# nh2/lz4-frame-conduit

Measured on AMD Instinct MI355X. Metric: GiB/s end-to-end (compress+decompress), 4 MiB blocks, 1/2/4/8 GPUs vs liblz4, higher is better.
Workload: dtype u8

## Files before the change

lz4_frame_conduit_amd/csrc/encode.cuh:

```cuda
#pragma once
#include <type_traits>
#include "common.cuh"

namespace lz4f {

constexpr uint32_t MFLIMIT = 12, LASTLIT = 5, MINMATCH = 4;
constexpr uint32_t ENC_POOL_SHORT = 0x200u;

struct ChunkInfo {
    uint32_t nrec;
    uint32_t first_lit;
    uint32_t tail_lit;
    uint32_t body_size;
    uint32_t carry_in;
    uint32_t flags;
    uint64_t out_off;
};

struct EncGeom {
    uint64_t src_size;
    uint64_t first_off;
    uint32_t write_endmark;
    uint32_t block_size;
    uint32_t chunk_size;
    uint32_t chunks_per_block;
    uint32_t n_blocks;
    uint32_t n_chunks;
    uint32_t linked;
    uint32_t block_checksum;
    uint32_t header_size;
    uint8_t  header[20];
    uint32_t max_rec_per_chunk;
    uint64_t rec_pool;
    uint32_t seed_stride;
    uint32_t tiles_per_wg;
    uint32_t e1_solo;
    uint32_t hc_attempts;
    uint32_t hc_lazy;
};

struct EncPlace {
    uint64_t bstart, bend_abs;
    uint64_t cs_abs, ce_abs;
    uint64_t low_abs;
    uint64_t rd_end;
};
__device__ __forceinline__ bool enc_place(const EncGeom& g, uint32_t chunk, EncPlace& pl)
{
    const uint32_t blk = chunk / g.chunks_per_block, cib = chunk % g.chunks_per_block;
    pl.bstart = g.first_off + (uint64_t)blk * g.block_size;
    pl.bend_abs = (pl.bstart + g.block_size < g.src_size) ? pl.bstart + g.block_size : g.src_size;
    pl.cs_abs = pl.bstart + (uint64_t)cib * g.chunk_size;
    if (pl.cs_abs >= pl.bend_abs) return false;
    pl.ce_abs = (pl.cs_abs + g.chunk_size < pl.bend_abs) ? pl.cs_abs + g.chunk_size : pl.bend_abs;
    pl.low_abs = g.linked ? 0 : pl.bstart;
    pl.rd_end = g.src_size;
    return true;
}

__device__ __forceinline__ unsigned long long* rec_ctl(const uint64_t* recs) { return (unsigned long long*)recs; }
__device__ __forceinline__ uint32_t* rec_offs(const uint64_t* recs) { return (uint32_t*)(recs + 8); }
__host__ __device__ __forceinline__ uint64_t rec_pool_at(uint32_t n_chunks) { return 8 + (((uint64_t)n_chunks + 1 + 15) / 16) * 8; }
__device__ __forceinline__ uint64_t* rec_pool_of(const uint64_t* recs, const EncGeom& g) { return (uint64_t*)recs + rec_pool_at(g.n_chunks); }

__device__ __forceinline__ uint32_t len_ext_bytes(uint32_t v) { return v >= 15 ? (v - 15) / 255 + 1 : 0; }
__device__ __forceinline__ uint32_t seq_size(uint32_t lit, uint32_t mlen)
{
    return 1 + len_ext_bytes(lit) + lit + 2 + len_ext_bytes(mlen - MINMATCH);
}
__device__ __forceinline__ uint64_t pack_rec(uint32_t lit, uint32_t mlen, uint32_t off)
{
    return (uint64_t)lit | ((uint64_t)mlen << 24) | ((uint64_t)off << 48);
}

struct uint4_ua { uint32_t x, y, z, w; } __attribute__((packed, aligned(1)));
__device__ __forceinline__ uint32_t ld32(const uint8_t* p) { return *(const u32_ua*)p; }
typedef uint64_t u64_ua __attribute__((aligned(1)));
__device__ __forceinline__ uint64_t ld64_guard(const uint8_t* p, const uint8_t* end)
{
    if (p + 8 <= end) return *(const u64_ua*)p;
    uint64_t v = 0;
    for (int i = 0; i < 8; i++) if (p + i < end) v |= (uint64_t)p[i] << (8 * i);
    return v;
}

constexpr uint32_t E1_TILE = 65536, E1_RING = 2 * E1_TILE, E1_RMASK = E1_RING - 1;
#ifndef E1_SLICE_BYTES
#define E1_SLICE_BYTES 128
#endif
constexpr uint32_t E1_SLICE = E1_SLICE_BYTES, E1_NSLICE = E1_TILE / E1_SLICE, E1_REC_PER_SLICE = E1_SLICE / MINMATCH;
constexpr uint32_t E1_HASH_LOG = 13;
#ifndef E1_WAVES
#define E1_WAVES 16
#endif
#ifdef E1_DEBUG
#define E1DBG(...) __VA_ARGS__
#else
#define E1DBG(...)
#endif
#define E1_DBG_AT (((uint64_t)gridDim.x) * (2 * E1_NSLICE * E1_REC_PER_SLICE))
struct alignas(16) E1Shared {
    uint16_t table[1u << E1_HASH_LOG];
    uint8_t  tags[1u << E1_HASH_LOG];
    uint32_t s_end[2][E1_NSLICE];
    uint8_t  s_n[2][E1_NSLICE];
    uint32_t next, cov;
    uint32_t first;
    uint32_t cur[16];
    uint32_t pieces[2];
    uint32_t mode, hits;
    uint32_t tail_d[2];
    uint32_t idle[64];
    alignas(16) uint8_t ring[E1_RING + 16];
};
static_assert(sizeof(E1Shared) <= 163840, "one workgroup per CU");
static_assert(64 * E1_WAVES >= E1_NSLICE, "a thread per slice when the lists are merged");
#ifndef E1_GRAB
#define E1_GRAB 8
#endif
#ifndef E1_GRAB_D
#define E1_GRAB_D 1
#endif
#ifndef E1_DENSE_PASS
#define E1_DENSE_PASS 1
#endif
#ifndef E1_V2
#define E1_V2 1
#endif
#ifndef E1_V3
#define E1_V3 1
#endif
#ifndef E1_V4
#define E1_V4 1
#endif
#ifndef E1_STEP0
#define E1_STEP0 4
#endif
#ifndef E1_IP2
#define E1_IP2 0
#endif
#ifndef E1_OPENER
#define E1_OPENER 2
#endif
#ifndef E1_ALIGN
#define E1_ALIGN 1
#endif
#ifndef E1_STEP_HIT
#define E1_STEP_HIT 1
#endif
constexpr uint32_t E1_GRAB_SPARSE = E1_GRAB, E1_GRAB_DENSE = E1_GRAB_D, E1_PROBE_SLICES = 16, E1_DENSE_HITS = 24;

struct __attribute__((aligned(4))) e1_w2 { uint32_t a, b; };
struct __attribute__((aligned(4))) e1_w3 { uint32_t a, b, c; };
__device__ __forceinline__ uint32_t e1_ld32(const uint8_t* ring, uint32_t pos)
{
    const uint32_t i = pos & E1_RMASK;
    const e1_w2 w = *(const e1_w2*)(ring + (i & ~3u));
    return __builtin_amdgcn_alignbyte(w.b, w.a, i & 3u);
}
__device__ __forceinline__ uint64_t e1_ld64(const uint8_t* ring, uint32_t pos)
{
    const uint32_t i = pos & E1_RMASK;
    const e1_w3 w = *(const e1_w3*)(ring + (i & ~3u));
    return (uint64_t)__builtin_amdgcn_alignbyte(w.b, w.a, i & 3u) | ((uint64_t)__builtin_amdgcn_alignbyte(w.c, w.b, i & 3u) << 32);
}
struct __attribute__((aligned(4))) e1_w5 { uint32_t a, b, c, d, e; };
__device__ __forceinline__ e1_w5 e1_ld5(const uint8_t* ring, uint32_t pos)
{
    return *(const e1_w5*)(ring + ((pos & E1_RMASK) & ~3u));
}
__device__ __forceinline__ uint32_t e1_same16(const e1_w5& s1, const e1_w5& s2, uint32_t k1, uint32_t k2)
{
    const uint32_t x0 = __builtin_amdgcn_alignbyte(s1.b, s1.a, k1) ^ __builtin_amdgcn_alignbyte(s2.b, s2.a, k2);
    const uint32_t x1 = __builtin_amdgcn_alignbyte(s1.c, s1.b, k1) ^ __builtin_amdgcn_alignbyte(s2.c, s2.b, k2);
    const uint32_t x2 = __builtin_amdgcn_alignbyte(s1.d, s1.c, k1) ^ __builtin_amdgcn_alignbyte(s2.d, s2.c, k2);
    const uint32_t x3 = __builtin_amdgcn_alignbyte(s1.e, s1.d, k1) ^ __builtin_amdgcn_alignbyte(s2.e, s2.d, k2);
    const uint64_t lo = (uint64_t)x0 | ((uint64_t)x1 << 32), hi = (uint64_t)x2 | ((uint64_t)x3 << 32);
    return lo ? (uint32_t)(__builtin_ctzll(lo) >> 3) : hi ? 8u + (uint32_t)(__builtin_ctzll(hi) >> 3) : 16u;
}
__device__ __forceinline__ uint32_t e1_mix(uint32_t v) { return v * 2654435761u; }
__device__ __forceinline__ uint32_t e1_slot(uint32_t hv) { return hv >> (32 - E1_HASH_LOG); }
__device__ __forceinline__ uint32_t e1_tag(uint32_t hv) { return (hv >> (24 - E1_HASH_LOG)) & 0xFFu; }
__device__ __forceinline__ uint32_t wave_excl_scan(uint32_t v, uint32_t& total)
{
    const uint32_t lane = lane_id();
    uint32_t incl = v;
#pragma unroll
    for (int sft = 1; sft < 64; sft <<= 1) { const uint32_t t = __shfl_up(incl, sft); if ((int)lane >= sft) incl += t; }
    total = __builtin_amdgcn_readlane(incl, 63);
    return incl - v;
}
__device__ __forceinline__ uint32_t wave_max(uint32_t v)
{
#pragma unroll
    for (int s = 1; s < 64; s <<= 1) { const uint32_t t = __shfl_xor(v, s); v = t > v ? t : v; }
    return v;
}
__device__ __forceinline__ uint32_t wave_sum(uint32_t v)
{
#pragma unroll
    for (int s = 1; s < 64; s <<= 1) v += __shfl_xor(v, s);
    return v;
}
__device__ __forceinline__ uint32_t wave_min16(uint32_t v)
{
    uint32_t t;
    t = (uint32_t)__builtin_amdgcn_update_dpp((int)v, (int)v, 0x111 , 0xf, 0xf, false); v = t < v ? t : v;
    t = (uint32_t)__builtin_amdgcn_update_dpp((int)v, (int)v, 0x112 , 0xf, 0xf, false); v = t < v ? t : v;
    t = (uint32_t)__builtin_amdgcn_update_dpp((int)v, (int)v, 0x114 , 0xf, 0xf, false); v = t < v ? t : v;
    t = (uint32_t)__builtin_amdgcn_update_dpp((int)v, (int)v, 0x118 , 0xf, 0xf, false); v = t < v ? t : v;
    return (uint32_t)__builtin_amdgcn_readlane((int)v, 15);
}
__device__ __forceinline__ uint32_t wave_excl_scan_max(uint32_t v)
{
    const uint32_t lane = lane_id();
    uint32_t incl = v;
#pragma unroll
    for (int sft = 1; sft < 64; sft <<= 1) { const uint32_t t = __shfl_up(incl, sft); if ((int)lane >= sft) incl = t > incl ? t : incl; }
    const uint32_t ex = __shfl_up(incl, 1);
    return lane == 0 ? 0u : ex;
}
constexpr uint32_t E1_PIECE_LOG = 12, E1_NPIECE = E1_TILE >> E1_PIECE_LOG;
__device__ __forceinline__ void e1_dma_piece(E1Shared& sh, const uint8_t* __restrict__ src, uint64_t org, uint32_t nts, uint32_t pc)
{
    const uint32_t lane = lane_id();
    const uint32_t ring0 = (uint32_t)(uintptr_t)(lptr_t)sh.ring;
#pragma unroll
    for (uint32_t q = 0; q < 4; q++) {
        const uint32_t at = nts + (pc << E1_PIECE_LOG) + q * 1024u;
        const uint8_t* gsrc = src + (org + at + lane * 16u);
        const uint32_t ldst = uni(ring0 + (at & E1_RMASK));
        uint32_t keep;
        asm volatile("s_mov_b32 %0, m0\n\ts_mov_b32 m0, %2\n\ts_nop 0\n\tglobal_load_lds_dwordx4 %1, off\n\ts_mov_b32 m0, %0" : "=&s"(keep) : "v"(gsrc), "s"(ldst) : "memory");
    }
}

__device__ __forceinline__ void e1_fill(E1Shared& sh, const uint8_t* __restrict__ src, uint64_t org, uint32_t a, uint32_t b, uint32_t tid)
{
    constexpr uint32_t NT = 64 * E1_WAVES;
    auto put = [&](uint32_t p) { const uint8_t v = src[org + p]; sh.ring[p & E1_RMASK] = v; if ((p & E1_RMASK) < 16) sh.ring[E1_RING + (p & E1_RMASK)] = v; };
    const uint32_t a16 = (a + 15u) & ~15u, b16 = b & ~15u;
    if (a16 < b16) {
        for (uint32_t u = a16 + tid * 16; u < b16; u += NT * 16) {
            const b16_ua t = *(const b16_ua*)(src + (org + u));
            const uint32_t i = u & E1_RMASK;
            *(uint4*)(sh.ring + i) = uint4{t.a, t.b, t.c, t.d};
            if (i == 0) *(uint4*)(sh.ring + E1_RING) = uint4{t.a, t.b, t.c, t.d};
        }
        if (tid < a16 - a) put(a + tid);
        if (tid < b - b16) put(b16 + tid);
    } else {
        for (uint32_t p = a + tid; p < b; p += NT) put(p);
    }
}

struct E1Walk {
    uint32_t pos, cov, bend;
    __device__ __forceinline__ bool step(uint64_t x, uint32_t& start, uint32_t& mlen)
    {
        const uint32_t lit = (uint32_t)(x & 0xFFFFFFu); mlen = (uint32_t)((x >> 24) & 0xFFFFFFu);
        start = pos + lit;
        const uint32_t end = start + mlen;
        pos = end;
        if (end <= cov) return false;
        if (start < cov) {
            const uint32_t ml2 = end - cov;
            if (ml2 < MINMATCH || cov + MFLIMIT > bend) return false;
            start = cov; mlen = ml2;
        }
        return true;
    }
};

__global__ __launch_bounds__(64 * E1_WAVES) void k_find_matches(const uint8_t* __restrict__ src, EncGeom g, ChunkInfo* __restrict__ info,
                                                                uint64_t* __restrict__ recs, uint64_t* __restrict__ scratch)
{
    __shared__ E1Shared sh;
    constexpr uint32_t NT = 64 * E1_WAVES;
    const uint32_t tid = threadIdx.x, lane = lane_id(), wave = uni(tid >> 6);
    uint64_t* spec = scratch + (uint64_t)blockIdx.x * (2 * E1_NSLICE * E1_REC_PER_SLICE);
    const uint32_t c0 = blockIdx.x * g.tiles_per_wg;
    const uint32_t c1 = (c0 + g.tiles_per_wg < g.n_chunks) ? c0 + g.tiles_per_wg : g.n_chunks;
    const uint64_t s0 = g.first_off + (uint64_t)c0 * E1_TILE;
    const uint64_t org = s0 - E1_TILE;
    uint32_t hist = 0, len0 = 0;
    if (s0 < g.src_size) {
        const uint64_t bstart0 = g.first_off + (uint64_t)(c0 / g.chunks_per_block) * g.block_size;
        const uint64_t bend0 = (bstart0 + g.block_size < g.src_size) ? bstart0 + g.block_size : g.src_size;
        const uint64_t low_abs = g.linked ? 0 : bstart0;
        hist = (uint32_t)((s0 - low_abs < E1_TILE) ? s0 - low_abs : E1_TILE);
        len0 = (uint32_t)((bend0 - s0 < E1_TILE) ? bend0 - s0 : E1_TILE);
    }
    const uint32_t hist0 = E1_TILE - hist;
    for (uint32_t i = tid; i < (1u << E1_HASH_LOG) / 2; i += NT) ((uint32_t*)sh.table)[i] = 0;
    for (uint32_t i = tid; i < (1u << E1_HASH_LOG) / 4; i += NT) ((uint32_t*)sh.tags)[i] = 0;
    e1_fill(sh, src, org, hist0, E1_TILE + len0, tid);
    __syncthreads();
    const uint32_t nt_seed = (g.e1_solo & 1u) ? WAVE : NT;
    if (tid < nt_seed) for (uint32_t p = hist0 + tid * g.seed_stride; p < E1_TILE; p += nt_seed * g.seed_stride)
        if (p + 4 <= E1_TILE + len0) { const uint32_t hv = e1_mix(e1_ld32(sh.ring, p)); sh.table[e1_slot(hv)] = (uint16_t)p; sh.tags[e1_slot(hv)] = (uint8_t)e1_tag(hv); }

    auto merge = [&](uint32_t c, uint32_t par, uint32_t ts, uint32_t te, uint32_t bend, uint32_t nslice) {
        constexpr uint32_t SP = E1_NSLICE / WAVE;
        const uint32_t* s_end = sh.s_end[par];
        const uint8_t* s_n = sh.s_n[par];
        const uint64_t* spc = spec + (size_t)par * (E1_NSLICE * E1_REC_PER_SLICE);
        const uint32_t s_lo = lane * SP;
        uint32_t lmax = 0;
#pragma unroll
        for (uint32_t j = 0; j < SP; j++) { const uint32_t e = (s_lo + j < nslice) ? s_end[s_lo + j] : 0u; lmax = e > lmax ? e : lmax; }
        uint32_t cov0 = wave_excl_scan_max(lmax);
        if (cov0 < ts) cov0 = ts;
        uint32_t nn[SP]; ulonglong2 x01[SP];
#pragma unroll
        for (uint32_t j = 0; j < SP; j++) nn[j] = (s_lo + j < nslice) ? s_n[s_lo + j] : 0u;
#pragma unroll
        for (uint32_t j = 0; j < SP; j++) x01[j] = *(const ulonglong2*)(spc + (nn[j] ? s_lo + j : 0u) * E1_REC_PER_SLICE);
        uint32_t kept = 0, f_start = 0, f_mlen = 0, last_end = 0, body = 0;
        {
            uint32_t cov = cov0;
#pragma unroll
            for (uint32_t j = 0; j < SP; j++) {
                const uint32_t sj = s_lo + j, n = nn[j];
                const uint64_t* lst = spc + sj * E1_REC_PER_SLICE;
                E1Walk w{ts + sj * E1_SLICE, cov, bend};
                ulonglong2 cur = x01[j];
                for (uint32_t r = 0; r < n; r += 2) {
                    ulonglong2 nx2 = cur;
                    if (r + 2 < n) nx2 = *(const ulonglong2*)(lst + r + 2);
#pragma unroll
                    for (uint32_t h = 0; h < 2; h++) {
                        if (r + h >= n) break;
                        uint32_t st, ml;
                        if (!w.step(h ? cur.y : cur.x, st, ml)) continue;
                        if (kept == 0) { f_start = st; f_mlen = ml; }
                        else body += seq_size(st - last_end, ml);
                        last_end = st + ml; kept++;
                    }
                    cur = nx2;
                }
                const uint32_t e = (sj < nslice) ? s_end[sj] : 0u; cov = e > cov ? e : cov;
            }
        }
        uint32_t ktot;
        uint32_t prev_end = wave_excl_scan_max(last_end);
        const uint32_t off = wave_excl_scan(kept, ktot);
        uint32_t kmax = wave_max(last_end);
        if (prev_end < ts) prev_end = ts;
        if (kmax < ts) kmax = ts;
        const uint32_t f_lit = kept ? f_start - prev_end : 0u;
        if (kept) body += seq_size(f_lit, f_mlen);
        const uint32_t btot = wave_sum(body);
        const uint64_t has = __ballot(kept != 0);
        const uint32_t tile_first = has ? (uint32_t)__builtin_amdgcn_readlane(f_lit, (int)__builtin_ctzll(has)) : 0u;
        unsigned long long base = 0;
        if (lane == 0 && ktot) base = atomicAdd(rec_ctl(recs), (unsigned long long)ktot);
        base = ((unsigned long long)__builtin_amdgcn_readfirstlane((uint32_t)(base >> 32)) << 32) | __builtin_amdgcn_readfirstlane((uint32_t)base);
        const bool room = base + ktot <= g.rec_pool;
        if (!room && lane == 0) atomicAdd(rec_ctl(recs) + 1, 1ull);
        if (room) {
            if (lane == 0) rec_offs(recs)[c] = (uint32_t)base;
            uint64_t* out = rec_pool_of(recs, g) + base + off;
            uint32_t cov = cov0, jn = 0, le = prev_end;
#pragma unroll
            for (uint32_t j = 0; j < SP; j++) {
                const uint32_t sj = s_lo + j, n = nn[j];
                const uint64_t* lst = spc + sj * E1_REC_PER_SLICE;
                E1Walk w{ts + sj * E1_SLICE, cov, bend};
                ulonglong2 cur = x01[j];
                for (uint32_t r = 0; r < n; r += 2) {
                    ulonglong2 nx2 = cur;
                    if (r + 2 < n) nx2 = *(const ulonglong2*)(lst + r + 2);
#pragma unroll
                    for (uint32_t h = 0; h < 2; h++) {
                        if (r + h >= n) break;
                        const uint64_t x = h ? cur.y : cur.x;
                        uint32_t st, ml;
                        if (!w.step(x, st, ml)) continue;
                        out[jn++] = pack_rec(st - le, ml, (uint32_t)(x >> 48));
                        le = st + ml;
                    }
                    cur = nx2;
                }
                const uint32_t e = (sj < nslice) ? s_end[sj] : 0u; cov = e > cov ? e : cov;
            }
        }
        ChunkInfo* ci = info + c;
        if (lane == 0) {
            if (room) { ci->nrec = ktot; ci->first_lit = tile_first; ci->tail_lit = te - kmax; ci->body_size = btot; }
            else      { ci->nrec = 0; ci->first_lit = 0; ci->tail_lit = te - ts; ci->body_size = 0; }
            sh.mode = (uint64_t)ktot * 64 > (uint64_t)(te - ts) ? 2u : 1u;
        }
    };

    if (tid == 0) { sh.mode = 0; sh.cov = E1_TILE; sh.hits = 0; sh.first = 0; sh.next = E1_ALIGN ? 0 : 1; sh.pieces[0] = 0; sh.pieces[1] = 0; sh.tail_d[0] = 0; sh.tail_d[1] = 0; }
    if (tid < 16) sh.cur[tid] = 0;
    uint32_t mode_tile = 0;
    uint32_t hold = 1;
    bool pend = false;
    uint32_t p_c = 0, p_par = 0, p_ts = 0, p_te = 0, p_bend = 0, p_ns = 0;
    __syncthreads();
    for (uint32_t c = c0; c < c1; c++) {
        const uint32_t k = c - c0;
        const uint32_t ts = E1_TILE * (k + 1), par = k & 1u;
        const uint32_t blk = c / g.chunks_per_block;
        const uint64_t bstart = g.first_off + (uint64_t)blk * g.block_size;
        const uint64_t bend_abs = (bstart + g.block_size < g.src_size) ? bstart + g.block_size : g.src_size;
        const uint64_t cs_abs = s0 + (uint64_t)k * E1_TILE;
        if (cs_abs >= bend_abs) {
            ChunkInfo* ci = info + c;
            if (tid == 0) { ci->nrec = 0; ci->first_lit = 0; ci->tail_lit = 0; ci->body_size = 0; }
            continue;
        }
        const uint32_t tlen = (uint32_t)((bend_abs - cs_abs < E1_TILE) ? bend_abs - cs_abs : E1_TILE);
        const uint32_t te = ts + tlen;
        const uint32_t bend = ts + (uint32_t)(bend_abs - cs_abs);
        const uint32_t blen = (uint32_t)(bend_abs - bstart);
        const uint32_t nslice = (tlen + E1_SLICE - 1) / E1_SLICE;
        uint32_t low = hist0;
        if (!g.linked) { const uint64_t back = cs_abs - bstart; if (back < (uint64_t)(ts - hist0)) low = ts - (uint32_t)back; }
        uint64_t* spec_t = spec + (size_t)par * (E1_NSLICE * E1_REC_PER_SLICE);

        uint32_t nlen = 0;
        const uint32_t nts = ts + E1_TILE;
        if (c + 1 < c1) {
            const uint32_t nblk = (c + 1) / g.chunks_per_block;
            const uint64_t nbstart = g.first_off + (uint64_t)nblk * g.block_size;
            const uint64_t nbend = (nbstart + g.block_size < g.src_size) ? nbstart + g.block_size : g.src_size;
            const uint64_t ncs = cs_abs + E1_TILE;
            if (ncs < nbend) nlen = (uint32_t)((nbend - ncs < E1_TILE) ? nbend - ncs : E1_TILE);
        }
        const bool nlen_full = nlen == E1_TILE;

        E1DBG(const unsigned long long q0 = clock64();)
        if (pend && wave == E1_WAVES - 1) {
            *(lane == 0 ? &sh.cur[wave] : &sh.idle[lane]) = 0xFFFFFFFFu;
            merge(p_c, p_par, p_ts, p_te, p_bend, p_ns);
        }

        E1DBG(const unsigned long long q1 = clock64();)
        const uint32_t end_lim = (te < bend - LASTLIT) ? te : bend - LASTLIT;
        E1DBG(uint32_t dq = 0; unsigned long long a_deq = 0, a_probe = 0, a_hit = 0, n_step = 0, n_hit = 0, n_deq = 0;)
        bool fresh = true;
        for (;;) {
            if ((g.e1_solo & 1u) && tid >= WAVE) break;
            E1DBG(const unsigned long long z0 = clock64(); n_deq++;)
            E1DBG(if (++dq > 100000) { if (lane == 0) atomicAdd((unsigned long long*)&scratch[E1_DBG_AT + 0], 1ull); break; })
            uint32_t mode = (g.e1_solo & 1u) ? mode_tile : uni(__hip_atomic_load(&sh.mode, __ATOMIC_RELAXED, __HIP_MEMORY_SCOPE_WORKGROUP));
            const bool opener = fresh && wave == 0 && (!E1_ALIGN || hold);
            const uint32_t grab = opener ? 1u : mode == 1 ? E1_GRAB_SPARSE : mode == 2 ? E1_GRAB_DENSE : 1u;
            uint32_t si = 0;
            if (E1_ALIGN && opener) si = uni(atomicAdd(lane == 0 ? &sh.next : &sh.idle[lane], grab));
            if (!opener) {
                if (fresh && E1_OPENER && ((E1_OPENER == 1 && !E1_ALIGN) || hold)) for (uint32_t spin = 0; spin < 4096 && uni(__hip_atomic_load(&sh.first, __ATOMIC_RELAXED, __HIP_MEMORY_SCOPE_WORKGROUP)) == 0; spin++) __builtin_amdgcn_s_sleep(2);
                si = uni(atomicAdd(lane == 0 ? &sh.next : &sh.idle[lane], grab));
            }
            fresh = false;
            if (si >= nslice) { *(lane == 0 ? &sh.cur[wave] : &sh.idle[lane]) = 0xFFFFFFFFu; break; }
            *(lane == 0 ? &sh.cur[wave] : &sh.idle[lane]) = si;
            if (nlen_full && (si & 31u) < grab) {
                uint32_t mn = lane < E1_WAVES ? __hip_atomic_load(&sh.cur[lane], __ATOMIC_RELAXED, __HIP_MEMORY_SCOPE_WORKGROUP) : 0xFFFFFFFFu;
                mn = wave_min16(mn);
                uint32_t ok_p = mn == 0xFFFFFFFFu ? 0u : (mn * E1_SLICE) >> E1_PIECE_LOG;
                if (ok_p > E1_NPIECE) ok_p = E1_NPIECE;
                const uint32_t had = uni(atomicMax(lane == 0 ? &sh.pieces[par] : &sh.idle[lane], ok_p));
                for (uint32_t pc = had; pc < ok_p; pc++) e1_dma_piece(sh, src, org, ts + E1_TILE, pc);
            }
            if (mode == 0 && si >= 2 * E1_PROBE_SLICES) {
                mode = uni(__hip_atomic_load(&sh.hits, __ATOMIC_RELAXED, __HIP_MEMORY_SCOPE_WORKGROUP)) > E1_DENSE_HITS ? 2u : 1u;
                *(lane == 0 ? &sh.mode : &sh.idle[lane]) = mode;
                mode_tile = mode;
            }
            const uint32_t cs = ts + si * E1_SLICE;
            const uint32_t ce = (cs + grab * E1_SLICE < te) ? cs + grab * E1_SLICE : te;
            uint64_t* myrec = spec_t + si * E1_REC_PER_SLICE;
            E1DBG(a_deq += clock64() - z0;)
            uint32_t nrec = 0, anchor = cs;
            uint32_t ip = uni(__hip_atomic_load(&sh.cov, __ATOMIC_RELAXED, __HIP_MEMORY_SCOPE_WORKGROUP));
            if (ip < cs) ip = cs;
            if (!(g.e1_solo & 2u) && blen >= MFLIMIT + 1 && ip + MINMATCH <= te && ip + MFLIMIT <= bend && ip < ce) {
                uint32_t last_start = ce - 1;
                if (te - MINMATCH < last_start) last_start = te - MINMATCH;
                if (bend - MFLIMIT < last_start) last_start = bend - MFLIMIT;
                const uint32_t floor_b = ip;
                uint32_t step = (E1_STEP0 > 1 && mode == 1 && !opener) ? (uint32_t)E1_STEP0 : 1u, two = opener ? 0u : 1u;
                E1DBG(uint32_t it = 0;)
                while (ip <= last_start) {
                    E1DBG(if (++it > 100000) { if (lane == 0) { atomicAdd((unsigned long long*)&scratch[E1_DBG_AT + 1], 1ull); scratch[E1_DBG_AT + 8] = ((uint64_t)ip << 32) | last_start; scratch[E1_DBG_AT + 9] = ((uint64_t)step << 32) | si; } break; })
                    E1DBG(const unsigned long long z1 = clock64(); n_step++;)
                    const uint32_t ipB = ip + WAVE * step, stepB = step + 1;
                    const uint32_t pA = ip + lane * step, pB = ipB + lane * stepB;
                    const bool actA = pA <= last_start, actB = two && pB <= last_start;
#if E1_V3
                    const uint32_t iA = pA & E1_RMASK, iB = pB & E1_RMASK;
                    const e1_w2 wA = *(const e1_w2*)(sh.ring + (iA & ~3u)), wB = *(const e1_w2*)(sh.ring + (iB & ~3u));
                    __builtin_amdgcn_sched_barrier(0);
                    const uint32_t vA = __builtin_amdgcn_alignbyte(wA.b, wA.a, iA & 3u), vB = __builtin_amdgcn_alignbyte(wB.b, wB.a, iB & 3u);
                    const uint32_t hvA = e1_mix(vA), hA = e1_slot(hvA), tgA = e1_tag(hvA);
                    const uint32_t hvB = e1_mix(vB), hB = e1_slot(hvB), tgB = e1_tag(hvB);
                    const uint32_t eA = sh.table[hA], etA = sh.tags[hA], eB = sh.table[hB], etB = sh.tags[hB];
                    __builtin_amdgcn_sched_barrier(0);
#else
                    const uint32_t vA = e1_ld32(sh.ring, pA), vB = e1_ld32(sh.ring, pB);
                    const uint32_t hvA = e1_mix(vA), hA = e1_slot(hvA), tgA = e1_tag(hvA);
                    const uint32_t hvB = e1_mix(vB), hB = e1_slot(hvB), tgB = e1_tag(hvB);
                    const uint32_t eA = sh.table[hA], etA = sh.tags[hA], eB = sh.table[hB], etB = sh.tags[hB];
#endif
                    const uint32_t distA = (pA - eA) & 0xFFFFu, distB = (pB - eB) & 0xFFFFu;
                    const uint32_t roomA = pA - low, roomB = pB - low;
#if E1_V3
                    const uint32_t xA = (uint32_t)(uint16_t)((uint16_t)distA - (uint16_t)1u) | ((etA ^ tgA) << 20);
                    const uint32_t xB = (uint32_t)(uint16_t)((uint16_t)distB - (uint16_t)1u) | ((etB ^ tgB) << 20);
#else
                    const uint32_t xA = ((distA - 1u) & 0xFFFFu) | ((etA ^ tgA) << 20) | (distA == 0u ? 1u << 19 : 0u);
                    const uint32_t xB = ((distB - 1u) & 0xFFFFu) | ((etB ^ tgB) << 20) | (distB == 0u ? 1u << 19 : 0u);
#endif
                    const uint32_t nbA = (uint32_t)__builtin_amdgcn_update_dpp(0, (int)vA, 0x111 , 0xf, 0xf, E1_V3 ? true : false);
                    const uint32_t nbB = (uint32_t)__builtin_amdgcn_update_dpp(0, (int)vB, 0x111 , 0xf, 0xf, E1_V3 ? true : false);
#if E1_V2
                    const uint64_t actmA = __ballot(pA <= last_start), actmB = __ballot(pB <= last_start) & (two ? ~0ull : 0ull);
                    constexpr uint32_t LIMCAP = E1_V3 ? 65535u : 65536u;
                    const uint32_t limA = roomA < LIMCAP ? roomA : LIMCAP, limB = roomB < LIMCAP ? roomB : LIMCAP;
                    const bool rleA = nbA == vA, rleB = nbB == vB;
                    const uint32_t dA = rleA ? step : distA, dB = rleB ? stepB : distB;
                    const uint32_t yA = rleA ? step - 1u : xA, yB = rleB ? stepB - 1u : xB;
                    uint64_t m = __ballot(yA < limA) & actmA;
                    if (m) m &= __ballot(e1_ld32(sh.ring, pA - dA) == vA);
                    bool inB = false;
                    if (!m) {
                        *(actA ? &sh.table[hA] : (uint16_t*)&sh.idle[lane]) = (uint16_t)pA; *(actA ? &sh.tags[hA] : (uint8_t*)&sh.idle[lane]) = (uint8_t)tgA;
                        m = __ballot(yB < limB) & actmB;
                        if (m) m &= __ballot(e1_ld32(sh.ring, pB - dB) == vB);
                        inB = true;
                    }
#else
                    const uint32_t limA = actA ? (roomA < 65536u ? roomA : 65536u) : 0u, limB = actB ? (roomB < 65536u ? roomB : 65536u) : 0u;
                    const uint32_t row0 = (lane & 15u) == 0u ? 1u : 0u;
                    uint64_t m = __ballot(xA < limA);
                    if (m) m &= __ballot(e1_ld32(sh.ring, pA - distA) == vA);
                    uint64_t mr = __ballot(((nbA ^ vA) | row0 | (actA ? 0u : 1u)) == 0u) & ~m;
                    m |= mr;
                    bool inB = false;
                    if (!m) {
                        *(actA ? &sh.table[hA] : (uint16_t*)&sh.idle[lane]) = (uint16_t)pA; *(actA ? &sh.tags[hA] : (uint8_t*)&sh.idle[lane]) = (uint8_t)tgA;
                        m = __ballot(xB < limB);
                        if (m) m &= __ballot(e1_ld32(sh.ring, pB - distB) == vB);
                        mr = __ballot(((nbB ^ vB) | row0 | (actB ? 0u : 1u)) == 0u) & ~m;
                        m |= mr;
                        inB = true;
                    }
                    const uint32_t dA = ((mr >> lane) & 1ull) ? step : distA, dB = ((mr >> lane) & 1ull) ? stepB : distB;
#endif
                    const uint32_t L = m ? (uint32_t)__builtin_ctzll(m) : WAVE;
                    {
                        const bool ins = (inB ? actB : actA) && lane <= L;
                        const uint32_t hI = inB ? hB : hA, pI = inB ? pB : pA, tI = inB ? tgB : tgA;
                        *(ins ? &sh.table[hI] : (uint16_t*)&sh.idle[lane]) = (uint16_t)pI; *(ins ? &sh.tags[hI] : (uint8_t*)&sh.idle[lane]) = (uint8_t)tI;
                    }
                    E1DBG(const unsigned long long z2 = clock64(); a_probe += z2 - z1;)
                    if (!m) { ip = two ? ipB + WAVE * stepB : ipB; step += 1 + two; two = 1; continue; }
                    E1DBG(n_hit++;)
                    if (E1_DENSE_PASS && !inB && mode == 2 && step == 1) {
                        const uint32_t di = dA;
                        const uint64_t x0 = e1_ld64(sh.ring, pA + 4) ^ e1_ld64(sh.ring, pA + 4 - di);
                        const uint64_t x1 = e1_ld64(sh.ring, pA + 12) ^ e1_ld64(sh.ring, pA + 12 - di);
                        const uint32_t xb = e1_ld32(sh.ring, pA - 4) ^ e1_ld32(sh.ring, pA - 4 - di);
                        const uint32_t g0 = x0 ? (uint32_t)(__builtin_ctzll(x0) >> 3) : 8u, g1 = x1 ? (uint32_t)(__builtin_ctzll(x1) >> 3) : 8u;
                        const uint32_t fraw = 4u + g0 + (g0 == 8u ? g1 : 0u), flim = end_lim - pA;
                        const uint32_t fl = fraw < flim ? fraw : flim;
                        const uint32_t lng = (fraw >= 20u && flim > 20u) ? 1u : 0u;
                        const uint32_t nbk = xb ? (uint32_t)(__builtin_clz(xb) >> 3) : 4u;
                        const uint32_t flx = fl | (lng << 31);
                        if (!((uint32_t)__builtin_amdgcn_readlane((int)flx, (int)L) >> 31)) {
                            uint64_t taken = 0, rem = m;
                            uint32_t endrel = 0, stop_at = WAVE;
                            for (;;) {
                                const uint32_t sx = (uint32_t)__builtin_ctzll(rem);
                                const uint32_t fx = (uint32_t)__builtin_amdgcn_readlane((int)flx, (int)sx);
                                if (fx >> 31) { stop_at = sx; break; }
                                taken |= 1ull << sx;
                                endrel = sx + fx;
                                if (endrel >= WAVE) break;
                                rem &= ~((1ull << endrel) - 1ull);
                                if (!rem) break;
                            }
                            const bool is_t = (taken >> lane) & 1ull;
                            const uint32_t pe = dpp_excl_scan_max(is_t ? lane + fl : 0u);
                            const uint32_t before = pe ? ip + pe : anchor;
                            const uint32_t bfloor = pe ? ip + pe : (anchor > floor_b ? anchor : floor_b);
                            uint32_t nb = nbk;
                            if (pA - bfloor < nb) nb = pA - bfloor;
                            if (pA - di - low < nb) nb = pA - di - low;
                            const uint32_t rank = (uint32_t)__builtin_popcountll(taken & ((1ull << lane) - 1ull));
                            if (is_t) myrec[nrec + rank] = pack_rec(pA - nb - before, fl + nb, di);
                            nrec += (uint32_t)__builtin_popcountll(taken);
                            E1DBG(if (blockIdx.x == 0 && lane == 0) { atomicAdd((unsigned long long*)&scratch[E1_DBG_AT + 13], 1ull); atomicAdd((unsigned long long*)&scratch[E1_DBG_AT + 14], (unsigned long long)__builtin_popcountll(taken)); atomicAdd((unsigned long long*)&scratch[E1_DBG_AT + 15], (unsigned long long)(stop_at < WAVE ? stop_at : (endrel > WAVE ? endrel : WAVE))); })
                            anchor = ip + endrel;
                            const uint32_t nrel = stop_at < WAVE ? stop_at : (endrel > WAVE ? endrel : WAVE);
                            const bool ins2 = actA && lane > L && lane < nrel && lane >= pe;
                            *(ins2 ? &sh.table[hA] : (uint16_t*)&sh.idle[lane]) = (uint16_t)pA; *(ins2 ? &sh.tags[hA] : (uint8_t*)&sh.idle[lane]) = (uint8_t)tgA;
                            ip += nrel;
                            atomicMax(lane == 0 ? &sh.cov : &sh.idle[lane], anchor);
                            step = 1; two = 1;
                            E1DBG(a_hit += clock64() - z2;)
                            continue;
                        }
                    }
                    E1DBG(if (blockIdx.x == 0 && lane == 0) { atomicAdd((unsigned long long*)&scratch[E1_DBG_AT + 4 + (inB ? 0 : mode != 2 ? 1 : step != 1 ? 2 : 3)], 1ull); })
                    const uint32_t dsel = inB ? dB : dA;
                    uint32_t mp = (uint32_t)__builtin_amdgcn_readlane(inB ? pB : pA, L);
                    const uint32_t d = (uint32_t)__builtin_amdgcn_readlane(dsel, L);
                    uint32_t room = mp - (anchor > floor_b ? anchor : floor_b); if (mp - d - low < room) room = mp - d - low;
                    uint32_t nb = 0;
                    E1DBG(uint32_t itb = 0;)
#if E1_V4
                    uint32_t fw = 0;
                    {
                        const uint32_t kb = lane + 1;
                        const uint32_t b1 = sh.ring[(mp - kb) & E1_RMASK], b2 = sh.ring[(mp - d - kb) & E1_RMASK];
                        const uint32_t a0 = mp + lane * 16;
                        const e1_w5 s1 = e1_ld5(sh.ring, a0), s2 = e1_ld5(sh.ring, a0 - d);
                        __builtin_amdgcn_sched_barrier(0);
                        const uint64_t ne = __ballot(b1 != b2 || kb > room);
                        nb = ne ? (uint32_t)__builtin_ctzll(ne) : WAVE;
                        uint32_t g0 = e1_same16(s1, s2, a0 & 3u, (a0 - d) & 3u);
                        const int32_t r = (int32_t)(end_lim - a0); g0 = r <= 0 ? 0u : (g0 > (uint32_t)r ? (uint32_t)r : g0);
                        const uint64_t stop = __ballot(g0 < 16);
                        if (stop) { const uint32_t f = (uint32_t)__builtin_ctzll(stop); fw = f * 16 + (uint32_t)__builtin_amdgcn_readlane(g0, f); }
                        else fw = WAVE * 16 | 0x80000000u;
                    }
                    for (bool more = nb == WAVE; more;) {
                        E1DBG(if (++itb > 100000) { if (lane == 0) { atomicAdd((unsigned long long*)&scratch[E1_DBG_AT + 2], 1ull); scratch[E1_DBG_AT + 10] = ((uint64_t)room << 32) | nb; } break; })
                        const uint32_t kb = nb + lane + 1;
                        const uint32_t b1 = sh.ring[(mp - kb) & E1_RMASK], b2 = sh.ring[(mp - d - kb) & E1_RMASK];
                        const uint64_t ne = __ballot(b1 != b2 || kb > room);
                        const uint32_t n1 = ne ? (uint32_t)__builtin_ctzll(ne) : WAVE;
                        nb += n1;
                        more = n1 == WAVE;
                    }
                    E1DBG(uint32_t itf = 0;)
                    while (fw >> 31) {
                        fw &= 0x7FFFFFFFu;
                        E1DBG(if (++itf > 100000) { if (lane == 0) { atomicAdd((unsigned long long*)&scratch[E1_DBG_AT + 3], 1ull); scratch[E1_DBG_AT + 11] = ((uint64_t)mp << 32) | fw; scratch[E1_DBG_AT + 12] = ((uint64_t)end_lim << 32) | d; } break; })
                        const uint32_t a0 = mp + fw + lane * 16;
                        const e1_w5 s1 = e1_ld5(sh.ring, a0), s2 = e1_ld5(sh.ring, a0 - d);
                        uint32_t g0 = e1_same16(s1, s2, a0 & 3u, (a0 - d) & 3u);
                        const int32_t r = (int32_t)(end_lim - a0); g0 = r <= 0 ? 0u : (g0 > (uint32_t)r ? (uint32_t)r : g0);
                        const uint64_t stop = __ballot(g0 < 16);
                        if (stop) { const uint32_t f = (uint32_t)__builtin_ctzll(stop); fw += f * 16 + (uint32_t)__builtin_amdgcn_readlane(g0, f); }
                        else fw = (fw + WAVE * 16) | 0x80000000u;
                    }
#else
                    for (;;) {
                        E1DBG(if (++itb > 100000) { if (lane == 0) { atomicAdd((unsigned long long*)&scratch[E1_DBG_AT + 2], 1ull); scratch[E1_DBG_AT + 10] = ((uint64_t)room << 32) | nb; } break; })
                        const uint32_t kb = nb + lane + 1;
                        const bool eq = kb <= room && sh.ring[(mp - kb) & E1_RMASK] == sh.ring[(mp - d - kb) & E1_RMASK];
                        const uint64_t ne = __ballot(!eq);
                        const uint32_t n1 = ne ? (uint32_t)__builtin_ctzll(ne) : WAVE;
                        nb += n1;
                        if (n1 < WAVE) break;
                    }
                    uint32_t fw = 0;
                    E1DBG(uint32_t itf = 0;)
                    for (;;) {
                        E1DBG(if (++itf > 100000) { if (lane == 0) { atomicAdd((unsigned long long*)&scratch[E1_DBG_AT + 3], 1ull); scratch[E1_DBG_AT + 11] = ((uint64_t)mp << 32) | fw; scratch[E1_DBG_AT + 12] = ((uint64_t)end_lim << 32) | d; } break; })
                        const uint32_t a0 = mp + fw + lane * 8;
                        uint32_t g0 = 0;
                        if (a0 < end_lim) {
                            const uint64_t x = e1_ld64(sh.ring, a0) ^ e1_ld64(sh.ring, a0 - d);
                            g0 = x ? (uint32_t)(__builtin_ctzll(x) >> 3) : 8u;
                            const uint32_t r = end_lim - a0; if (g0 > r) g0 = r;
                        }
                        const uint64_t stop = __ballot(g0 < 8);
                        if (stop) { const uint32_t f = (uint32_t)__builtin_ctzll(stop); fw += f * 8 + (uint32_t)__builtin_amdgcn_readlane(g0, f); break; }
                        fw += WAVE * 8;
                    }
#endif
                    mp -= nb;
                    const uint32_t mlen = nb + fw;
                    myrec[nrec] = pack_rec(mp - anchor, mlen, d);
                    nrec++;
                    anchor = ip = mp + mlen;
                    step = (E1_STEP_HIT > 1 && mode == 1) ? (uint32_t)E1_STEP_HIT : 1u; two = 1;
                    atomicMax(lane == 0 ? &sh.cov : &sh.idle[lane], ip);
                    if (E1_OPENER == 2) *((lane == 0 && ip == end_lim) ? &sh.tail_d[par] : &sh.idle[lane]) = d;
                    E1DBG(a_hit += clock64() - z2;)
                    if (E1_IP2 && ip >= low + 2 && ip + 2 <= te) { const uint32_t q2 = ip - 2, hv2 = e1_mix(e1_ld32(sh.ring, q2)); *(lane == 0 ? &sh.table[e1_slot(hv2)] : (uint16_t*)&sh.idle[lane]) = (uint16_t)q2; *(lane == 0 ? &sh.tags[e1_slot(hv2)] : (uint8_t*)&sh.idle[lane]) = (uint8_t)e1_tag(hv2); }
                }
            }
            const bool mine_s = lane < grab && si + lane < nslice;
            *(mine_s ? &sh.s_end[par][si + lane] : &sh.idle[lane]) = (lane == 0 && nrec) ? anchor : 0u;
            *(mine_s ? &sh.s_n[par][si + lane] : (uint8_t*)&sh.idle[lane]) = (uint8_t)(lane == 0 ? nrec : 0u);
            if (mode == 0) atomicAdd(lane == 0 ? &sh.hits : &sh.idle[lane], nrec);
            if (opener) *(lane == 0 ? &sh.first : &sh.idle[lane]) = 1u;
        }
        E1DBG(const unsigned long long q2 = clock64();)
        __builtin_amdgcn_s_waitcnt(0);
        __syncthreads();
        mode_tile = uni(__hip_atomic_load(&sh.mode, __ATOMIC_RELAXED, __HIP_MEMORY_SCOPE_WORKGROUP));
        E1DBG(const unsigned long long q3 = clock64();)
        pend = true; p_c = c; p_par = par; p_ts = ts; p_te = te; p_bend = bend; p_ns = nslice;

        if (tid == 0) { sh.tail_d[par ^ 1u] = 0; sh.cov = nts; sh.hits = 0; sh.first = 0; sh.next = E1_ALIGN ? 0 : 1; sh.pieces[par ^ 1u] = 0; }
        if (tid < 16) sh.cur[tid] = 0;
        if (nlen) {
            if (nlen_full) {
                const uint32_t had = sh.pieces[par];
                for (uint32_t pc = had + wave; pc < E1_NPIECE; pc += E1_WAVES) e1_dma_piece(sh, src, org, nts, pc);
                if ((nts & E1_RMASK) == 0 && tid >= 64 && tid < 68) ((uint32_t*)(sh.ring + E1_RING))[tid - 64] = *(const u32_ua*)(src + (org + nts + (tid - 64) * 4u));
            } else e1_fill(sh, src, org, nts, nts + nlen, tid);
        }
        E1DBG(const unsigned long long q4 = clock64();)
        asm volatile("s_waitcnt vmcnt(0)" ::: "memory");
        E1DBG(const unsigned long long q5 = clock64();)
        __syncthreads();
        {
            const uint32_t td = uni(__hip_atomic_load(&sh.tail_d[par], __ATOMIC_RELAXED, __HIP_MEMORY_SCOPE_WORKGROUP));
            hold = (g.e1_solo & 1u) || (td != 0 && nlen >= 4 && uni(e1_ld32(sh.ring, nts)) == uni(e1_ld32(sh.ring, nts - td))) ? 1u : 0u;
        }
        E1DBG(if (blockIdx.x == 0 && lane == 0) { unsigned long long* d = (unsigned long long*)&scratch[E1_DBG_AT + 16 + wave * 8]; d[0] += q1 - q0; d[1] += q2 - q1; d[2] += q3 - q2; d[3] += q4 - q3; d[4] += q5 - q4; d[5] += clock64() - q5; d[6] += 1; unsigned long long* f = (unsigned long long*)&scratch[E1_DBG_AT + 160 + wave * 6]; f[0] += a_deq; f[1] += a_probe; f[2] += a_hit; f[3] += n_deq; f[4] += n_step; f[5] += n_hit; })
    }
    if (pend && wave == E1_WAVES - 1) merge(p_c, p_par, p_ts, p_te, p_bend, p_ns);
}


__device__ __forceinline__ uint32_t layout_block_chunks(ChunkInfo* __restrict__ ci, const uint32_t nch, const uint32_t blen)
{
    const uint32_t lane = lane_id();
    uint32_t carry_run = 0, total = 0;
    for (uint32_t c0 = 0; c0 < nch; c0 += WAVE) {
        const uint32_t c = c0 + lane;
        const bool act = c < nch;
        const uint4 x = act ? *(const uint4*)&ci[c] : uint4{0u, 0u, 0u, 0u};
        const bool has = act && x.x != 0;
        const uint64_t m = __ballot(has);
        uint32_t sum_tail, sum_size;
        const uint32_t pt = wave_excl_scan(act ? x.z : 0u, sum_tail);
        const uint64_t below = m & ((1ull << lane) - 1ull);
        const uint32_t p = below ? 63u - (uint32_t)__builtin_clzll(below) : 0u;
        const uint32_t pt_p = __shfl(pt, (int)p);
        const uint32_t carry = below ? pt - pt_p : carry_run + pt;
        const uint32_t size = has ? x.w + carry + len_ext_bytes(x.y + carry) - len_ext_bytes(x.y) : 0u;
        const uint32_t off = wave_excl_scan(size, sum_size);
        if (act) {
            *(uint2*)&ci[c].carry_in = uint2{carry, (c + 1 == nch) ? 2u : 0u};
            ci[c].out_off = total + off;
        }
        if (m) { const uint32_t last = 63u - (uint32_t)__builtin_clzll(m); carry_run = sum_tail - (uint32_t)__shfl(pt, (int)last); }
        else carry_run += sum_tail;
        total += sum_size;
    }
    total += 1 + len_ext_bytes(carry_run) + carry_run;
    const bool raw = total >= blen;
    if (raw) for (uint32_t c = lane; c < nch; c += WAVE) ci[c].flags = ((c + 1 == nch) ? 2u : 0u) | 1u;
    return raw ? (blen | 0x80000000u) : total;
}
__device__ __forceinline__ void layout_block(const EncGeom& g, ChunkInfo* __restrict__ info, BlockOut* __restrict__ table, uint32_t* __restrict__ blk_bytes, uint32_t b)
{
    const uint64_t bstart = g.first_off + (uint64_t)b * g.block_size;
    const uint32_t blen = (uint32_t)((bstart + g.block_size < g.src_size) ? g.block_size : g.src_size - bstart);
    const uint32_t word = layout_block_chunks(info + (uint64_t)b * g.chunks_per_block, (blen + g.chunk_size - 1) / g.chunk_size, blen);
    if (lane_id() == 0) {
        table[b].word = word;
        table[b].dst_off = bstart - g.first_off;
        table[b].dst_size = blen;
        blk_bytes[b] = 4 + (word & 0x7FFFFFFFu) + 4 * g.block_checksum;
    }
}
template <int WAVES_PER_WG>
__global__ __launch_bounds__(64 * WAVES_PER_WG) void k_layout_blocks(EncGeom g, ChunkInfo* __restrict__ info, BlockOut* __restrict__ table,
                                                                     uint32_t* __restrict__ blk_bytes)
{
    const uint32_t b = uni(blockIdx.x * WAVES_PER_WG + (threadIdx.x >> 6));
    if (b >= g.n_blocks) return;
    layout_block(g, info, table, blk_bytes, b);
}

__device__ __forceinline__ void layout_scan(const EncGeom& g, BlockOut* __restrict__ table, const uint32_t* __restrict__ blk_bytes,
                                            uint8_t* __restrict__ dst, uint64_t dst_cap, ResultRec* __restrict__ res, const uint64_t* __restrict__ recs,
                                            uint64_t* s_part, uint64_t& s_carry)
{
    const uint32_t t = threadIdx.x;
    if (t == 0) s_carry = g.header_size;
    __syncthreads();
    for (uint32_t base = 0; base < g.n_blocks; base += 1024) {
        const uint32_t b = base + t;
        const uint64_t v = (b < g.n_blocks) ? blk_bytes[b] : 0;
        s_part[t] = v;
        __syncthreads();
        for (uint32_t off = 1; off < 1024; off <<= 1) {
            uint64_t add = (t >= off) ? s_part[t - off] : 0;
            __syncthreads();
            s_part[t] += add;
            __syncthreads();
        }
        if (b < g.n_blocks) table[b].src_off = s_carry + s_part[t] - v + 4;
        __syncthreads();
        if (t == 1023) s_carry += s_part[1023];
        __syncthreads();
    }
    const uint64_t frame_size = s_carry + (g.write_endmark == 2 ? 8 : g.write_endmark ? 4 : 0);
    const bool fits = frame_size <= dst_cap;
    if (fits) {
        if (t < g.header_size) dst[t] = g.header[t];
        if (t < 4 && g.write_endmark) dst[s_carry + t] = 0;
    }
    if (t == 0 && res) {
        res->size = fits ? frame_size : 0; res->consumed = g.src_size - g.first_off;
        res->status = fits ? ST_OK : ST_DSTSMALL; res->n_blocks = g.n_blocks; res->first_bad_block = 0xFFFFFFFFu; res->flags = g.header[4] | ((g.n_chunks && rec_ctl(recs)[1]) ? ENC_POOL_SHORT : 0u);
    }
    if (t == 0 && g.n_chunks) { rec_ctl(recs)[0] = 0ull; rec_ctl(recs)[1] = 0ull; }
}
__global__ __launch_bounds__(1024) void k_layout_scan(EncGeom g, BlockOut* __restrict__ table, const uint32_t* __restrict__ blk_bytes,
                                                      uint8_t* __restrict__ dst, uint64_t dst_cap, ResultRec* __restrict__ res, const uint64_t* __restrict__ recs)
{
    __shared__ uint64_t s_part[1024];
    __shared__ uint64_t s_carry;
    layout_scan(g, table, blk_bytes, dst, dst_cap, res, recs, s_part, s_carry);
}

__device__ __forceinline__ void layout_chunk(const EncGeom& g, ChunkInfo* __restrict__ info, const BlockOut* __restrict__ table,
                                             uint8_t* __restrict__ dst, const ResultRec* res, uint32_t chunk)
{
    if (res->status != ST_OK) { info[chunk].flags |= 4u; return; }
    const uint32_t b = chunk / g.chunks_per_block, c = chunk % g.chunks_per_block;
    const BlockOut e = table[b];
    const uint32_t nch = (e.dst_size + g.chunk_size - 1) / g.chunk_size;
    if (c == 0) { const uint32_t w = e.word; uint8_t* q = dst + e.src_off - 4; q[0] = (uint8_t)w; q[1] = (uint8_t)(w >> 8); q[2] = (uint8_t)(w >> 16); q[3] = (uint8_t)(w >> 24); }
    if (c >= nch) return;
    info[chunk].out_off = (e.word >> 31) ? e.src_off + (uint64_t)c * g.chunk_size : e.src_off + info[chunk].out_off;
}
__global__ __launch_bounds__(256) void k_layout_chunks(EncGeom g, ChunkInfo* __restrict__ info, const BlockOut* __restrict__ table,
                                                       uint8_t* __restrict__ dst, const ResultRec* __restrict__ res)
{
    const uint32_t chunk = blockIdx.x * 256 + threadIdx.x;
    if (chunk >= g.n_chunks) return;
    layout_chunk(g, info, table, dst, res, chunk);
}
constexpr uint32_t LAYOUT_SMALL_BLOCKS = 64, LAYOUT_SMALL_CHUNKS = 4096;
__global__ __launch_bounds__(1024) void k_layout_small(EncGeom g, ChunkInfo* info, BlockOut* table, uint32_t* blk_bytes, uint8_t* __restrict__ dst, uint64_t dst_cap,
                                                       ResultRec* res, const uint64_t* __restrict__ recs)
{
    __shared__ uint64_t s_part[1024];
    __shared__ uint64_t s_carry;
    for (uint32_t b = uni(threadIdx.x >> 6); b < g.n_blocks; b += 16) layout_block(g, info, table, blk_bytes, b);
    __threadfence_block(); __syncthreads();
    layout_scan(g, table, blk_bytes, dst, dst_cap, res, recs, s_part, s_carry);
// ... 424 lines not shown
```

Before: 757.7.

## Add fast sparse-mode slice claiming path and CAS-aligned grabs in encoder work queue

```diff
diff --git a/lz4_frame_conduit_amd/csrc/encode.cuh b/lz4_frame_conduit_amd/csrc/encode.cuh
--- a/lz4_frame_conduit_amd/csrc/encode.cuh
+++ b/lz4_frame_conduit_amd/csrc/encode.cuh
@@ -133,6 +133,12 @@
 #ifndef E1_V4
 #define E1_V4 1
 #endif
+#ifndef E1_V5
+#define E1_V5 1
+#endif
+#ifndef E1_V6
+#define E1_V6 1
+#endif
 #ifndef E1_STEP0
 #define E1_STEP0 4
 #endif
@@ -149,6 +155,7 @@
 #define E1_STEP_HIT 1
 #endif
 constexpr uint32_t E1_GRAB_SPARSE = E1_GRAB, E1_GRAB_DENSE = E1_GRAB_D, E1_PROBE_SLICES = 16, E1_DENSE_HITS = 24;
+static_assert((E1_GRAB_SPARSE & (E1_GRAB_SPARSE - 1u)) == 0, "a long helping's size is a power of two: its claims are aligned by masking");
 
 struct __attribute__((aligned(4))) e1_w2 { uint32_t a, b; };
 struct __attribute__((aligned(4))) e1_w3 { uint32_t a, b, c; };
@@ -442,22 +449,13 @@
         const uint32_t end_lim = (te < bend - LASTLIT) ? te : bend - LASTLIT;
         E1DBG(uint32_t dq = 0; unsigned long long a_deq = 0, a_probe = 0, a_hit = 0, n_step = 0, n_hit = 0, n_deq = 0;)
         bool fresh = true;
-        for (;;) {
-            if ((g.e1_solo & 1u) && tid >= WAVE) break;
-            E1DBG(const unsigned long long z0 = clock64(); n_deq++;)
-            E1DBG(if (++dq > 100000) { if (lane == 0) atomicAdd((unsigned long long*)&scratch[E1_DBG_AT + 0], 1ull); break; })
-            uint32_t mode = (g.e1_solo & 1u) ? mode_tile : uni(__hip_atomic_load(&sh.mode, __ATOMIC_RELAXED, __HIP_MEMORY_SCOPE_WORKGROUP));
-            const bool opener = fresh && wave == 0 && (!E1_ALIGN || hold);
-            const uint32_t grab = opener ? 1u : mode == 1 ? E1_GRAB_SPARSE : mode == 2 ? E1_GRAB_DENSE : 1u;
-            uint32_t si = 0;
-            if (E1_ALIGN && opener) si = uni(atomicAdd(lane == 0 ? &sh.next : &sh.idle[lane], grab));
-            if (!opener) {
-                if (fresh && E1_OPENER && ((E1_OPENER == 1 && !E1_ALIGN) || hold)) for (uint32_t spin = 0; spin < 4096 && uni(__hip_atomic_load(&sh.first, __ATOMIC_RELAXED, __HIP_MEMORY_SCOPE_WORKGROUP)) == 0; spin++) __builtin_amdgcn_s_sleep(2);
-                si = uni(atomicAdd(lane == 0 ? &sh.next : &sh.idle[lane], grab));
-            }
-            fresh = false;
-            if (si >= nslice) { *(lane == 0 ? &sh.cur[wave] : &sh.idle[lane]) = 0xFFFFFFFFu; break; }
-            *(lane == 0 ? &sh.cur[wave] : &sh.idle[lane]) = si;
+        E1DBG(unsigned long long z0 = 0;)
+#if E1_V5
+        const uint32_t lim_t = (!(g.e1_solo & 2u) && blen >= MFLIMIT + 1) ? ((te - MINMATCH < bend - MFLIMIT) ? te - MINMATCH : bend - MFLIMIT) : 0u;
+        const bool tile_plain = !(E1_ALIGN && mode_tile == 1u && !(g.e1_solo & 1u));
+        bool plain = tile_plain || hold;
+#endif
+        auto release = [&](const uint32_t si, const uint32_t grab) __attribute__((always_inline)) {
             if (nlen_full && (si & 31u) < grab) {
                 uint32_t mn = lane < E1_WAVES ? __hip_atomic_load(&sh.cur[lane], __ATOMIC_RELAXED, __HIP_MEMORY_SCOPE_WORKGROUP) : 0xFFFFFFFFu;
                 mn = wave_min16(mn);
@@ -466,22 +464,24 @@
                 const uint32_t had = uni(atomicMax(lane == 0 ? &sh.pieces[par] : &sh.idle[lane], ok_p));
                 for (uint32_t pc = had; pc < ok_p; pc++) e1_dma_piece(sh, src, org, ts + E1_TILE, pc);
             }
-            if (mode == 0 && si >= 2 * E1_PROBE_SLICES) {
-                mode = uni(__hip_atomic_load(&sh.hits, __ATOMIC_RELAXED, __HIP_MEMORY_SCOPE_WORKGROUP)) > E1_DENSE_HITS ? 2u : 1u;
-                *(lane == 0 ? &sh.mode : &sh.idle[lane]) = mode;
-                mode_tile = mode;
-            }
+        };
+        auto helping = [&](const uint32_t si, uint32_t ip, const uint32_t mode, const uint32_t grab, const bool opener) __attribute__((always_inline)) {
             const uint32_t cs = ts + si * E1_SLICE;
-            const uint32_t ce = (cs + grab * E1_SLICE < te) ? cs + grab * E1_SLICE : te;
             uint64_t* myrec = spec_t + si * E1_REC_PER_SLICE;
             E1DBG(a_deq += clock64() - z0;)
             uint32_t nrec = 0, anchor = cs;
-            uint32_t ip = uni(__hip_atomic_load(&sh.cov, __ATOMIC_RELAXED, __HIP_MEMORY_SCOPE_WORKGROUP));
             if (ip < cs) ip = cs;
+#if E1_V5
+            {
+                uint32_t last_start = cs + grab * E1_SLICE - 1u;
+                if (lim_t < last_start) last_start = lim_t;
+#else
+            const uint32_t ce = (cs + grab * E1_SLICE < te) ? cs + grab * E1_SLICE : te;
             if (!(g.e1_solo & 2u) && blen >= MFLIMIT + 1 && ip + MINMATCH <= te && ip + MFLIMIT <= bend && ip < ce) {
                 uint32_t last_start = ce - 1;
                 if (te - MINMATCH < last_start) last_start = te - MINMATCH;
                 if (bend - MFLIMIT < last_start) last_start = bend - MFLIMIT;
+#endif
                 const uint32_t floor_b = ip;
                 uint32_t step = (E1_STEP0 > 1 && mode == 1 && !opener) ? (uint32_t)E1_STEP0 : 1u, two = opener ? 0u : 1u;
                 E1DBG(uint32_t it = 0;)
@@ -693,6 +693,56 @@
             *(mine_s ? &sh.s_n[par][si + lane] : (uint8_t*)&sh.idle[lane]) = (uint8_t)(lane == 0 ? nrec : 0u);
             if (mode == 0) atomicAdd(lane == 0 ? &sh.hits : &sh.idle[lane], nrec);
             if (opener) *(lane == 0 ? &sh.first : &sh.idle[lane]) = 1u;
+        };
+        for (;;) {
+            if ((g.e1_solo & 1u) && tid >= WAVE) break;
+            E1DBG(z0 = clock64(); n_deq++;)
+            E1DBG(if (++dq > 100000) { if (lane == 0) atomicAdd((unsigned long long*)&scratch[E1_DBG_AT + 0], 1ull); break; })
+#if E1_V5
+            if (!plain) {
+                const uint32_t a = atomicAdd(lane == 0 ? &sh.next : &sh.idle[lane], E1_GRAB_SPARSE);
+                const uint32_t cv = __hip_atomic_load(&sh.cov, __ATOMIC_RELAXED, __HIP_MEMORY_SCOPE_WORKGROUP);
+                __builtin_amdgcn_sched_barrier(0);
+                const uint32_t si = uni(a);
+                if (si >= nslice) { *(lane == 0 ? &sh.cur[wave] : &sh.idle[lane]) = 0xFFFFFFFFu; break; }
+                *(lane == 0 ? &sh.cur[wave] : &sh.idle[lane]) = si;
+                release(si, E1_GRAB_SPARSE);
+                helping(si, uni(cv), 1u, E1_GRAB_SPARSE, false);
+                continue;
+            }
+            plain = tile_plain;
+#endif
+            uint32_t mode = (g.e1_solo & 1u) ? mode_tile : uni(__hip_atomic_load(&sh.mode, __ATOMIC_RELAXED, __HIP_MEMORY_SCOPE_WORKGROUP));
+            const bool opener = fresh && wave == 0 && (!E1_ALIGN || hold);
+            uint32_t grab = opener ? 1u : mode == 1 ? E1_GRAB_SPARSE : mode == 2 ? E1_GRAB_DENSE : 1u;
+            uint32_t si = 0;
+            if (E1_ALIGN && opener) si = uni(atomicAdd(lane == 0 ? &sh.next : &sh.idle[lane], grab));
+            if (!opener) {
+                if (fresh && E1_OPENER && ((E1_OPENER == 1 && !E1_ALIGN) || hold)) for (uint32_t spin = 0; spin < 4096 && uni(__hip_atomic_load(&sh.first, __ATOMIC_RELAXED, __HIP_MEMORY_SCOPE_WORKGROUP)) == 0; spin++) __builtin_amdgcn_s_sleep(2);
+                bool got = false;
+#if E1_V6
+                if (E1_ALIGN && mode == 1) {
+                    uint32_t n = uni(__hip_atomic_load(&sh.next, __ATOMIC_RELAXED, __HIP_MEMORY_SCOPE_WORKGROUP));
+                    for (uint32_t t = 0; t < 64 && !got; t++) {
+                        const uint32_t tgt = (n & ~(E1_GRAB_SPARSE - 1u)) + E1_GRAB_SPARSE;
+                        const uint32_t old = uni(atomicCAS(lane == 0 ? &sh.next : &sh.idle[lane], n, tgt));
+                        if (old == n) { got = true; si = n; grab = tgt - n; }
+                        n = old;
+                    }
+                }
+#endif
+                if (!got) si = uni(atomicAdd(lane == 0 ? &sh.next : &sh.idle[lane], grab));
+            }
+            fresh = false;
+            if (si >= nslice) { *(lane == 0 ? &sh.cur[wave] : &sh.idle[lane]) = 0xFFFFFFFFu; break; }
+            *(lane == 0 ? &sh.cur[wave] : &sh.idle[lane]) = si;
+            release(si, grab);
+            if (mode == 0 && si >= 2 * E1_PROBE_SLICES) {
+                mode = uni(__hip_atomic_load(&sh.hits, __ATOMIC_RELAXED, __HIP_MEMORY_SCOPE_WORKGROUP)) > E1_DENSE_HITS ? 2u : 1u;
+                *(lane == 0 ? &sh.mode : &sh.idle[lane]) = mode;
+                mode_tile = mode;
+            }
+            helping(si, uni(__hip_atomic_load(&sh.cov, __ATOMIC_RELAXED, __HIP_MEMORY_SCOPE_WORKGROUP)), mode, grab, opener);
         }
         E1DBG(const unsigned long long q2 = clock64();)
         __builtin_amdgcn_s_waitcnt(0);
```

Result: faster. 771.7, median of 6 (+1.8%).
